# RobotLocomotion/pytorch-dense-correspondence

Hardware: NVIDIA H100
Metric: image-pairs/s (640x480, D=3) fwd+loss+bwd (higher is better)
Workload: dtype f32 (bf16x3 split on the wgmma tensor cores, fp32 accumulate)

## Files before the change

### pytorch-dense-correspondence_b200/csrc/conv_tc.cu

```cuda
#include <cuda.h>
#include <algorithm>
#include <cstring>
#include <functional>
#include <mutex>
#include <unordered_map>

#include "conv.cuh"
#include "conv_tc.cuh"

namespace ddn {

constexpr int TC_BLOCK_K = 64;
constexpr int TC_CONSUMERS = 256;
constexpr int TC_THREADS = TC_CONSUMERS + 32;
constexpr int TC_PRODUCER_WARP = TC_CONSUMERS / 32;
constexpr int TC_WIDE_THREADS = TC_CONSUMERS + 128;
constexpr int TC_A_BYTES = 128 * TC_BLOCK_K * 2;

__device__ __forceinline__ uint32_t smem_u32(const void* p) { return (uint32_t)__cvta_generic_to_shared(p); }

__device__ __forceinline__ void mbar_init(uint32_t bar, uint32_t count) {
  asm volatile("mbarrier.init.shared::cta.b64 [%0], %1;" ::"r"(bar), "r"(count));
}
__device__ __forceinline__ void mbar_expect_tx(uint32_t bar, uint32_t bytes) {
// ... 24 lines not shown
  asm volatile(
      "cp.async.bulk.tensor.2d.shared::cluster.global.mbarrier::complete_tx::bytes [%0], [%1, {%3, %4}], [%2];"
      ::"r"(dst), "l"(map), "r"(bar), "r"(c0), "r"(c1) : "memory");
}
__device__ __forceinline__ void tma_prefetch_l2_4d(const CUtensorMap* map, int c0, int c1, int c2, int c3) {
  asm volatile("cp.async.bulk.prefetch.tensor.4d.L2.global.tile [%0, {%1, %2, %3, %4}];" ::"l"(map), "r"(c0), "r"(c1), "r"(c2), "r"(c3) : "memory");
}
__device__ __forceinline__ void tma_prefetch_desc(const CUtensorMap* map) {
  asm volatile("prefetch.tensormap [%0];" ::"l"(map) : "memory");
}

__device__ __forceinline__ uint64_t gmma_desc(uint32_t smem_addr, uint32_t lbo_bytes, uint32_t sbo_bytes) {
  return (uint64_t)((smem_addr >> 4) & 0x3FFF) | ((uint64_t)((lbo_bytes >> 4) & 0x3FFF) << 16) |
         ((uint64_t)((sbo_bytes >> 4) & 0x3FFF) << 32) | ((uint64_t)1 << 62);
}
__device__ __forceinline__ uint64_t gmma_desc_k(uint32_t smem_addr, uint32_t sbo_bytes = 1024) { return gmma_desc(smem_addr, 16, sbo_bytes); }

template <int R>
__device__ __forceinline__ void setmaxnreg_dec() { asm volatile("setmaxnreg.dec.sync.aligned.u32 %0;" ::"n"(R)); }
template <int R>
__device__ __forceinline__ void setmaxnreg_inc() { asm volatile("setmaxnreg.inc.sync.aligned.u32 %0;" ::"n"(R)); }
__device__ __forceinline__ void wgmma_fence() { asm volatile("wgmma.fence.sync.aligned;" ::: "memory"); }
__device__ __forceinline__ void wgmma_commit() { asm volatile("wgmma.commit_group.sync.aligned;" ::: "memory"); }
template <int N>
__device__ __forceinline__ void wgmma_wait() { asm volatile("wgmma.wait_group.sync.aligned %0;" ::"n"(N) : "memory"); }
template <int K>
__device__ __forceinline__ void fence_acc(float (&d)[K]) {
#pragma unroll
  for (int i = 0; i < K; ++i) asm volatile("" : "+f"(d[i])::"memory");
}

template <int N> struct Wgmma;
template <> struct Wgmma<32> {
  template <int TRANS>
  static __device__ __forceinline__ void mma(float (&d)[16], uint64_t a, uint64_t b, int scale_d) {
    asm volatile(
        "{\n.reg .pred p;\nsetp.ne.b32 p, %18, 0;\n"
        "wgmma.mma_async.sync.aligned.m64n32k16.f32.bf16.bf16 {"
        "%0, %1, %2, %3, %4, %5, %6, %7, %8, %9, %10, %11, %12, %13, %14, %15"
        "}, %16, %17, p, 1, 1, %19, %19;\n}\n"
        : "+f"(d[0]), "+f"(d[1]), "+f"(d[2]), "+f"(d[3]), "+f"(d[4]), "+f"(d[5]), "+f"(d[6]), "+f"(d[7]),
          "+f"(d[8]), "+f"(d[9]), "+f"(d[10]), "+f"(d[11]), "+f"(d[12]), "+f"(d[13]), "+f"(d[14]), "+f"(d[15])
        : "l"(a), "l"(b), "r"(scale_d), "n"(TRANS));
  }
};
template <> struct Wgmma<64> {
  template <int TRANS>
  static __device__ __forceinline__ void mma(float (&d)[32], uint64_t a, uint64_t b, int scale_d) {
    asm volatile(
        "{\n.reg .pred p;\nsetp.ne.b32 p, %34, 0;\n"
        "wgmma.mma_async.sync.aligned.m64n64k16.f32.bf16.bf16 {"
        "%0, %1, %2, %3, %4, %5, %6, %7, %8, %9, %10, %11, %12, %13, %14, %15, "
        "%16, %17, %18, %19, %20, %21, %22, %23, %24, %25, %26, %27, %28, %29, %30, %31"
        "}, %32, %33, p, 1, 1, %35, %35;\n}\n"
        : "+f"(d[0]), "+f"(d[1]), "+f"(d[2]), "+f"(d[3]), "+f"(d[4]), "+f"(d[5]), "+f"(d[6]), "+f"(d[7]),
          "+f"(d[8]), "+f"(d[9]), "+f"(d[10]), "+f"(d[11]), "+f"(d[12]), "+f"(d[13]), "+f"(d[14]), "+f"(d[15]),
          "+f"(d[16]), "+f"(d[17]), "+f"(d[18]), "+f"(d[19]), "+f"(d[20]), "+f"(d[21]), "+f"(d[22]), "+f"(d[23]),
          "+f"(d[24]), "+f"(d[25]), "+f"(d[26]), "+f"(d[27]), "+f"(d[28]), "+f"(d[29]), "+f"(d[30]), "+f"(d[31])
        : "l"(a), "l"(b), "r"(scale_d), "n"(TRANS));
  }
};
template <> struct Wgmma<128> {
  template <int TRANS>
  static __device__ __forceinline__ void mma(float (&d)[64], uint64_t a, uint64_t b, int scale_d) {
    asm volatile(
        "{\n.reg .pred p;\nsetp.ne.b32 p, %66, 0;\n"
        "wgmma.mma_async.sync.aligned.m64n128k16.f32.bf16.bf16 {"
        "%0, %1, %2, %3, %4, %5, %6, %7, %8, %9, %10, %11, %12, %13, %14, %15, "
        "%16, %17, %18, %19, %20, %21, %22, %23, %24, %25, %26, %27, %28, %29, %30, %31, "
        "%32, %33, %34, %35, %36, %37, %38, %39, %40, %41, %42, %43, %44, %45, %46, %47, "
        "%48, %49, %50, %51, %52, %53, %54, %55, %56, %57, %58, %59, %60, %61, %62, %63"
        "}, %64, %65, p, 1, 1, %67, %67;\n}\n"
        : "+f"(d[0]), "+f"(d[1]), "+f"(d[2]), "+f"(d[3]), "+f"(d[4]), "+f"(d[5]), "+f"(d[6]), "+f"(d[7]),
          "+f"(d[8]), "+f"(d[9]), "+f"(d[10]), "+f"(d[11]), "+f"(d[12]), "+f"(d[13]), "+f"(d[14]), "+f"(d[15]),
          "+f"(d[16]), "+f"(d[17]), "+f"(d[18]), "+f"(d[19]), "+f"(d[20]), "+f"(d[21]), "+f"(d[22]), "+f"(d[23]),
          "+f"(d[24]), "+f"(d[25]), "+f"(d[26]), "+f"(d[27]), "+f"(d[28]), "+f"(d[29]), "+f"(d[30]), "+f"(d[31]),
          "+f"(d[32]), "+f"(d[33]), "+f"(d[34]), "+f"(d[35]), "+f"(d[36]), "+f"(d[37]), "+f"(d[38]), "+f"(d[39]),
          "+f"(d[40]), "+f"(d[41]), "+f"(d[42]), "+f"(d[43]), "+f"(d[44]), "+f"(d[45]), "+f"(d[46]), "+f"(d[47]),
          "+f"(d[48]), "+f"(d[49]), "+f"(d[50]), "+f"(d[51]), "+f"(d[52]), "+f"(d[53]), "+f"(d[54]), "+f"(d[55]),
          "+f"(d[56]), "+f"(d[57]), "+f"(d[58]), "+f"(d[59]), "+f"(d[60]), "+f"(d[61]), "+f"(d[62]), "+f"(d[63])
        : "l"(a), "l"(b), "r"(scale_d), "n"(TRANS));
  }
};

template <int N, int TRANS, int NPROD>
__device__ __forceinline__ void mma_k16(float (&d)[N / 2], uint64_t a_hi, uint64_t a_lo, uint64_t b_hi, uint64_t b_lo, int accumulate) {
  if (NPROD == 3) {
    Wgmma<N>::template mma<TRANS>(d, a_hi, b_lo, accumulate);
    Wgmma<N>::template mma<TRANS>(d, a_lo, b_hi, 1);
    Wgmma<N>::template mma<TRANS>(d, a_hi, b_hi, 1);
  } else {
    Wgmma<N>::template mma<TRANS>(d, a_hi, b_hi, accumulate);
  }
}
template <int N, int TRANS, int NPROD>
__device__ __forceinline__ void mma_k16_x(float (&d)[N / 2], float (&x)[N / 2], uint64_t a_hi, uint64_t a_lo, uint64_t b_hi, uint64_t b_lo,
                                          int accumulate) {
  if (NPROD == 3) {
    Wgmma<N>::template mma<TRANS>(x, a_hi, b_lo, accumulate);
    Wgmma<N>::template mma<TRANS>(x, a_lo, b_hi, 1);
  }
  Wgmma<N>::template mma<TRANS>(d, a_hi, b_hi, accumulate);
}
template <int K>
__device__ __forceinline__ void add_cross(float (&d)[K], const float (&x)[K]) {
#pragma unroll
  for (int i = 0; i < K; ++i) d[i] += x[i];
}
template <int N, int K>
__device__ __forceinline__ float (&acc_cols(float (&d)[K]))[N / 2] {
  static_assert(N / 2 <= K, "accumulator too narrow");
  return *reinterpret_cast<float(*)[N / 2]>(&d[0]);
}

constexpr int EPI_ROWS = 4;
constexpr int EPI_STRIDE = 40;
constexpr int EPI_WARP_FLOATS = 16 * EPI_STRIDE;

template <int K>
__device__ __forceinline__ void stage_write(const float (&acc)[K], int c, float* st, int lane) {
  const int r = lane >> 2, q = (lane & 3) * 2;
#pragma unroll
  for (int jj = 0; jj < 4; ++jj) {
    const int j = 4 * c + jj;
    *reinterpret_cast<float2*>(st + r * EPI_STRIDE + 8 * jj + q) = make_float2(acc[4 * j], acc[4 * j + 1]);
    *reinterpret_cast<float2*>(st + (r + 8) * EPI_STRIDE + 8 * jj + q) = make_float2(acc[4 * j + 2], acc[4 * j + 3]);
  }
  __syncwarp();
}

template <int K>
__device__ __forceinline__ void stage_chunk(const float (&acc)[K], int c, float* st, int lane, float4 (&v)[EPI_ROWS]) {
  stage_write(acc, c, st, lane);
  const int ga = lane >> 3, gb = lane & 7;
#pragma unroll
  for (int i = 0; i < EPI_ROWS; ++i) v[i] = *reinterpret_cast<const float4*>(st + (EPI_ROWS * ga + i) * EPI_STRIDE + 4 * gb);
  __syncwarp();
}

__device__ __forceinline__ uint32_t pack_bf16x2(__nv_bfloat16 a, __nv_bfloat16 b) {
  return (uint32_t)__bfloat16_as_ushort(a) | ((uint32_t)__bfloat16_as_ushort(b) << 16);
}

struct TcEpilogueParams {
  float* out;
  const float* addend;
  int imgs_per_group;
  BnFwdFinal fin;
  TcBwdStats bst;
  const float* ep_scale; const float* ep_shift; int ep_relu;
  __nv_bfloat16* out_hi; __nv_bfloat16* out_lo;
};

__device__ __forceinline__ void conv_epilogue_rows(const TcEpilogueParams& p, const float4 (&v)[EPI_ROWS], size_t off, size_t rs, int n_ok, int ch,
                                                   int C, int grp, float4& s1, float4& s2) {
  float4 adv[EPI_ROWS];
#pragma unroll
  for (int i = 0; i < EPI_ROWS; ++i)
    adv[i] = (p.addend && i < n_ok) ? __ldg(reinterpret_cast<const float4*>(p.addend + off + i * rs)) : make_float4(0.f, 0.f, 0.f, 0.f);
  if (p.ep_scale) {
    const float4 sc = __ldg(reinterpret_cast<const float4*>(p.ep_scale + ch));
    const float4 sh = __ldg(reinterpret_cast<const float4*>(p.ep_shift + ch));
#pragma unroll
    for (int i = 0; i < EPI_ROWS; ++i) {
      float4 f = make_float4(fmaf(v[i].x, sc.x, sh.x) + adv[i].x, fmaf(v[i].y, sc.y, sh.y) + adv[i].y,
                             fmaf(v[i].z, sc.z, sh.z) + adv[i].z, fmaf(v[i].w, sc.w, sh.w) + adv[i].w);
      if (p.ep_relu) { f.x = fmaxf(f.x, 0.f); f.y = fmaxf(f.y, 0.f); f.z = fmaxf(f.z, 0.f); f.w = fmaxf(f.w, 0.f); }
      if (i < n_ok) {
        if (p.out) *reinterpret_cast<float4*>(p.out + off + i * rs) = f;
        if (p.out_hi) {
          const __nv_bfloat16 h0 = __float2bfloat16_rn(f.x), h1 = __float2bfloat16_rn(f.y), h2 = __float2bfloat16_rn(f.z), h3 = __float2bfloat16_rn(f.w);
          *reinterpret_cast<uint2*>(p.out_hi + off + i * rs) = make_uint2(pack_bf16x2(h0, h1), pack_bf16x2(h2, h3));
          if (p.out_lo)
            *reinterpret_cast<uint2*>(p.out_lo + off + i * rs) =
                make_uint2(pack_bf16x2(__float2bfloat16_rn(f.x - __bfloat162float(h0)), __float2bfloat16_rn(f.y - __bfloat162float(h1))),
                           pack_bf16x2(__float2bfloat16_rn(f.z - __bfloat162float(h2)), __float2bfloat16_rn(f.w - __bfloat162float(h3))));
        }
      }
    }
  } else if (p.bst.fin.a.acc) {
    float4 rw[EPI_ROWS];
    uint2 yh[EPI_ROWS];
#pragma unroll
    for (int i = 0; i < EPI_ROWS; ++i) {
      rw[i] = i < n_ok ? __ldg(reinterpret_cast<const float4*>(p.bst.raw + off + i * rs)) : make_float4(0.f, 0.f, 0.f, 0.f);
      if (p.bst.y_hi) yh[i] = i < n_ok ? __ldg(reinterpret_cast<const uint2*>(p.bst.y_hi + off + i * rs)) : make_uint2(0u, 0u);
    }
    const float4 mu = __ldg(reinterpret_cast<const float4*>(p.bst.mean + (size_t)grp * C + ch));
    const float4 is = __ldg(reinterpret_cast<const float4*>(p.bst.invstd + (size_t)grp * C + ch));
    float4 scl = make_float4(0.f, 0.f, 0.f, 0.f), be = scl;
    if (!p.bst.y_hi && p.bst.relu) {
      const float4 gm = __ldg(reinterpret_cast<const float4*>(p.bst.gamma + ch));
      be = __ldg(reinterpret_cast<const float4*>(p.bst.beta + ch));
      scl = make_float4(gm.x * is.x, gm.y * is.y, gm.z * is.z, gm.w * is.w);
    }
#pragma unroll
    for (int i = 0; i < EPI_ROWS; ++i) {
      float4 g = make_float4(v[i].x + adv[i].x, v[i].y + adv[i].y, v[i].z + adv[i].z, v[i].w + adv[i].w);
      if (i < n_ok) *reinterpret_cast<float4*>(p.out + off + i * rs) = g;
      else g = make_float4(0.f, 0.f, 0.f, 0.f);
      if (p.bst.y_hi) {
        const uint2 hh = yh[i];
        if ((hh.x & 0x8000u) || !(hh.x & 0x7fffu)) g.x = 0.f;
        if ((hh.x & 0x80000000u) || !(hh.x & 0x7fff0000u)) g.y = 0.f;
        if ((hh.y & 0x8000u) || !(hh.y & 0x7fffu)) g.z = 0.f;
        if ((hh.y & 0x80000000u) || !(hh.y & 0x7fff0000u)) g.w = 0.f;
      } else if (p.bst.relu) {
        if (!(fmaf(rw[i].x - mu.x, scl.x, be.x) > 0.f)) g.x = 0.f;
        if (!(fmaf(rw[i].y - mu.y, scl.y, be.y) > 0.f)) g.y = 0.f;
        if (!(fmaf(rw[i].z - mu.z, scl.z, be.z) > 0.f)) g.z = 0.f;
        if (!(fmaf(rw[i].w - mu.w, scl.w, be.w) > 0.f)) g.w = 0.f;
      }
      s1.x += g.x; s1.y += g.y; s1.z += g.z; s1.w += g.w;
      s2.x = fmaf(g.x, (rw[i].x - mu.x) * is.x, s2.x); s2.y = fmaf(g.y, (rw[i].y - mu.y) * is.y, s2.y);
      s2.z = fmaf(g.z, (rw[i].z - mu.z) * is.z, s2.z); s2.w = fmaf(g.w, (rw[i].w - mu.w) * is.w, s2.w);
    }
  } else {
#pragma unroll
    for (int i = 0; i < EPI_ROWS; ++i) {
      const float4 raw = i < n_ok ? v[i] : make_float4(0.f, 0.f, 0.f, 0.f);
      if (i < n_ok)
        *reinterpret_cast<float4*>(p.out + off + i * rs) = make_float4(raw.x + adv[i].x, raw.y + adv[i].y, raw.z + adv[i].z, raw.w + adv[i].w);
      s1.x += raw.x; s1.y += raw.y; s1.z += raw.z; s1.w += raw.w;
      s2.x = fmaf(raw.x, raw.x, s2.x); s2.y = fmaf(raw.y, raw.y, s2.y); s2.z = fmaf(raw.z, raw.z, s2.z); s2.w = fmaf(raw.w, raw.w, s2.w);
    }
  }
}

__device__ __forceinline__ void colsum_lane_groups(float4& s1, float4& s2) {
#pragma unroll
  for (int off = 8; off < 32; off <<= 1) {
    s1.x += __shfl_xor_sync(0xffffffffu, s1.x, off); s1.y += __shfl_xor_sync(0xffffffffu, s1.y, off);
    s1.z += __shfl_xor_sync(0xffffffffu, s1.z, off); s1.w += __shfl_xor_sync(0xffffffffu, s1.w, off);
    s2.x += __shfl_xor_sync(0xffffffffu, s2.x, off); s2.y += __shfl_xor_sync(0xffffffffu, s2.y, off);
    s2.z += __shfl_xor_sync(0xffffffffu, s2.z, off); s2.w += __shfl_xor_sync(0xffffffffu, s2.w, off);
  }
}

__device__ __forceinline__ void named_barrier(int id, int threads) { asm volatile("bar.sync %0, %1;" ::"r"(id), "r"(threads) : "memory"); }

__device__ __forceinline__ void conv_epilogue_finalize(const TcEpilogueParams& p, int C, int* s_last, int bar) {
  if (p.fin.a.acc) {
    if (bn_last_cta(p.fin.a.ticket, gridDim.x, threadIdx.x == 0, s_last, [bar] { named_barrier(bar, TC_CONSUMERS); }))
      for (int c = threadIdx.x; c < C; c += TC_CONSUMERS) bn_fwd_finalize_channel(p.fin, c);
  } else if (p.bst.fin.a.acc) {
    if (bn_last_cta(p.bst.fin.a.ticket, gridDim.x, threadIdx.x == 0, s_last, [bar] { named_barrier(bar, TC_CONSUMERS); }))
      for (int c = threadIdx.x; c < C; c += TC_CONSUMERS) bn_bwd_finalize_channel(p.bst.fin, c);
  }
}

struct TcConvParams {
  TcEpilogueParams epi;
  int N, H, W, Cin, Cout;
  int taps_w;
  int dil;
  int stride;
  int tiles_h, tiles_w;
  int n_sub;
  int n_co;
  int full_items, tail_split, total_items;
};

constexpr int TC_SUB_H = 4, TC_SUB_W = 16;
constexpr int TC_SUB_BYTES = 64 * 128;

struct TcItem { int sp, co0, width; };
__device__ __forceinline__ TcItem tc_item(const TcConvParams& p, int idx, int block_n) {
  int tile = idx, piece = 0, width = block_n;
  if (idx >= p.full_items) {
    const int j = idx - p.full_items;
    tile = p.full_items + j / p.tail_split;
    piece = j - (j / p.tail_split) * p.tail_split;
    width = block_n / p.tail_split;
  }
  TcItem it;
  it.sp = tile / p.n_co;
  it.co0 = (tile - it.sp * p.n_co) * block_n + piece * width;
  it.width = width;
  return it;
}
struct TcSub { int n, h0, w0; bool valid; };
__device__ __forceinline__ TcSub tc_sub(const TcConvParams& p, int st) {
  TcSub s;
  s.valid = st < p.n_sub;
  const int tw = st % p.tiles_w; const int t = st / p.tiles_w;
  const int th = t % p.tiles_h;
  s.n = s.valid ? t / p.tiles_h : p.N;
  s.h0 = th * TC_SUB_H; s.w0 = tw * TC_SUB_W;
  return s;
}

template <int W, int BLOCK_N, int NPROD, int STAGES, int TRANS = 0>
__device__ __forceinline__ void conv_tc_mainloop(float (&acc)[W / 2], float (&accx)[W / 2], int num_kb, uint32_t& g, const uint64_t* full_bar,
                                                 const uint64_t* empty_bar, const uint8_t* smem, int wg, int lane) {
  constexpr int NSPLIT = NPROD == 3 ? 2 : 1;
  constexpr int A_BYTES = 128 * TC_BLOCK_K * 2;
  constexpr int B_BYTES = BLOCK_N * TC_BLOCK_K * 2;
  constexpr int STAGE_BYTES = NSPLIT * (A_BYTES + B_BYTES);
  constexpr uint32_t LBO = TRANS ? TC_SUB_BYTES : 16;
  constexpr int K_STEP = TRANS ? 16 * 128 : 32;
  for (int kb = 0; kb < num_kb; ++kb, ++g) {
    const int s = g % STAGES;
    mbar_wait(smem_u32(&full_bar[s]), (g / STAGES) & 1);
    wgmma_fence();
    const uint32_t stg = smem_u32(smem + (size_t)s * STAGE_BYTES);
    const uint64_t a_hi = gmma_desc(stg + wg * TC_SUB_BYTES, LBO, 1024), a_lo = gmma_desc(stg + A_BYTES + wg * TC_SUB_BYTES, LBO, 1024);
    const uint64_t b_hi = gmma_desc(stg + NSPLIT * A_BYTES, LBO, 1024), b_lo = gmma_desc(stg + 2 * A_BYTES + B_BYTES, LBO, 1024);
#pragma unroll
    for (int k = 0; k < TC_BLOCK_K / 16; ++k) {
      const uint64_t adv = (uint64_t)((k * K_STEP) >> 4);
      mma_k16_x<W, TRANS, NPROD>(acc, accx, a_hi + adv, a_lo + adv, b_hi + adv, b_lo + adv, (kb | k) != 0);
    }
    wgmma_commit();
    wgmma_wait<1>();
    if (kb > 0 && lane == 0) mbar_arrive(smem_u32(&empty_bar[(g - 1) % STAGES]));
  }
  wgmma_wait<0>();
  fence_acc(acc);
  if (NPROD == 3) { fence_acc(accx); add_cross(acc, accx); }
  if (lane == 0) mbar_arrive(smem_u32(&empty_bar[(g - 1) % STAGES]));
}

template <int BLOCK_N, int NPROD>
__global__ void __launch_bounds__(TC_WIDE_THREADS, 1)
conv_tc_kernel(const __grid_constant__ CUtensorMap tm_a_hi, const __grid_constant__ CUtensorMap tm_a_lo,
               const __grid_constant__ CUtensorMap tm_b_hi, const __grid_constant__ CUtensorMap tm_b_lo,
               const __grid_constant__ CUtensorMap tm_bt_hi, const __grid_constant__ CUtensorMap tm_bt_lo,
               const TcConvParams p) {
  constexpr int NSPLIT = NPROD == 3 ? 2 : 1;
  constexpr int A_BYTES = 128 * TC_BLOCK_K * 2;
  constexpr int B_BYTES = BLOCK_N * TC_BLOCK_K * 2;
  constexpr int STAGE_BYTES = NSPLIT * (A_BYTES + B_BYTES);
  constexpr int STAGES = (192 * 1024) / STAGE_BYTES >= 8 ? 8 : (192 * 1024) / STAGE_BYTES;
  static_assert(STAGES >= 2, "pipeline needs at least two stages");

  extern __shared__ __align__(1024) uint8_t smem_raw[];
  uint8_t* smem = reinterpret_cast<uint8_t*>((reinterpret_cast<uintptr_t>(smem_raw) + 1023) & ~uintptr_t(1023));
  __shared__ __align__(8) uint64_t full_bar[STAGES];
  __shared__ __align__(8) uint64_t empty_bar[STAGES];
  __shared__ int s_last;
  __shared__ __align__(16) float s_stage[TC_CONSUMERS / 32][EPI_WARP_FLOATS];
  __shared__ __align__(16) float s_part[2][2][4][BLOCK_N];

  pdl_trigger();
  const int warp = __shfl_sync(0xffffffffu, threadIdx.x >> 5, 0), lane = threadIdx.x & 31;
  const int cin_chunks = p.Cin / TC_BLOCK_K;
  const int num_kb = p.taps_w * p.taps_w * cin_chunks;
  const int half = p.taps_w >> 1;

  if (threadIdx.x == 0) {
    for (int s = 0; s < STAGES; ++s) { mbar_init(smem_u32(&full_bar[s]), 1); mbar_init(smem_u32(&empty_bar[s]), TC_CONSUMERS / 32); }
    fence_barrier_init();
    tma_prefetch_desc(&tm_a_hi); tma_prefetch_desc(&tm_b_hi); tma_prefetch_desc(&tm_bt_hi);
    if (NSPLIT == 2) { tma_prefetch_desc(&tm_a_lo); tma_prefetch_desc(&tm_b_lo); tma_prefetch_desc(&tm_bt_lo); }
  }
  __syncthreads();
  pdl_wait();

  if (warp >= TC_PRODUCER_WARP) {
    setmaxnreg_dec<40>();
    if (warp == TC_PRODUCER_WARP && lane == 0) {
      uint32_t g = 0;
      for (int idx = blockIdx.x; idx < p.total_items; idx += gridDim.x) {
        const TcItem it = tc_item(p, idx, BLOCK_N);
        const bool tail = it.width != BLOCK_N;
        const uint32_t stage_tx = (uint32_t)(NSPLIT * (A_BYTES + it.width * TC_BLOCK_K * 2));
        const CUtensorMap* mb_hi = tail ? &tm_bt_hi : &tm_b_hi;
        const CUtensorMap* mb_lo = tail ? &tm_bt_lo : &tm_b_lo;
        const TcSub s0 = tc_sub(p, it.sp * 2), s1 = tc_sub(p, it.sp * 2 + 1);
        for (int kb = 0; kb < num_kb; ++kb, ++g) {
          const int s = g % STAGES;
          mbar_wait(smem_u32(&empty_bar[s]), ((g / STAGES) & 1) ^ 1);
          const int tap = kb / cin_chunks, cc = kb - tap * cin_chunks;
          const int r = tap / p.taps_w, sx = tap - r * p.taps_w;
          const int dh = (r - half) * p.dil, dw = (sx - half) * p.dil;
          uint8_t* stg = smem + (size_t)s * STAGE_BYTES;
          const uint32_t bar = smem_u32(&full_bar[s]);
          mbar_expect_tx(bar, stage_tx);
          tma_load_4d(smem_u32(stg), &tm_a_hi, bar, cc * TC_BLOCK_K, s0.w0 * p.stride + dw, s0.h0 * p.stride + dh, s0.n);
          tma_load_4d(smem_u32(stg + TC_SUB_BYTES), &tm_a_hi, bar, cc * TC_BLOCK_K, s1.w0 * p.stride + dw, s1.h0 * p.stride + dh, s1.n);
          tma_load_2d(smem_u32(stg + NSPLIT * A_BYTES), mb_hi, bar, kb * TC_BLOCK_K, it.co0);
          if (NSPLIT == 2) {
            tma_load_4d(smem_u32(stg + A_BYTES), &tm_a_lo, bar, cc * TC_BLOCK_K, s0.w0 * p.stride + dw, s0.h0 * p.stride + dh, s0.n);
            tma_load_4d(smem_u32(stg + A_BYTES + TC_SUB_BYTES), &tm_a_lo, bar, cc * TC_BLOCK_K, s1.w0 * p.stride + dw, s1.h0 * p.stride + dh, s1.n);
            tma_load_2d(smem_u32(stg + 2 * A_BYTES + B_BYTES), mb_lo, bar, kb * TC_BLOCK_K, it.co0);
          }
        }
      }
    }
  } else {
    setmaxnreg_inc<232>();
    const int wg = warp >> 2, w = warp & 3, e = threadIdx.x & 127;
    const int ga = lane >> 3, gb = lane & 7;
    const bool stats = p.epi.fin.a.acc != nullptr;
    const bool bstats = p.epi.bst.fin.a.acc != nullptr;
    double* const sum_acc = bstats ? p.epi.bst.fin.a.acc : p.epi.fin.a.acc;
    float* const st = s_stage[warp];
    float acc[BLOCK_N / 2], accx[BLOCK_N / 2];
    uint32_t g = 0;
    for (int idx = blockIdx.x; idx < p.total_items; idx += gridDim.x) {
      const TcItem it = tc_item(p, idx, BLOCK_N);
      if (it.width == BLOCK_N)
        conv_tc_mainloop<BLOCK_N, BLOCK_N, NPROD, STAGES>(acc, accx, num_kb, g, full_bar, empty_bar, smem, wg, lane);
      else if (BLOCK_N > 64 && it.width == 64)
        conv_tc_mainloop<64, BLOCK_N, NPROD, STAGES>(acc_cols<64>(acc), acc_cols<64>(accx), num_kb, g, full_bar, empty_bar, smem, wg, lane);
      else
        conv_tc_mainloop<32, BLOCK_N, NPROD, STAGES>(acc_cols<32>(acc), acc_cols<32>(accx), num_kb, g, full_bar, empty_bar, smem, wg, lane);

      const TcSub sb = tc_sub(p, it.sp * 2 + wg);
      const int h = sb.h0 + w, w4 = sb.w0 + EPI_ROWS * ga;
      const int n_ok = (sb.valid && h < p.H) ? min(EPI_ROWS, p.W - w4) : 0;
      const size_t pix = ((size_t)(n_ok > 0 ? sb.n : 0) * p.H + (n_ok > 0 ? h : 0)) * p.W + (n_ok > 0 ? w4 : 0);
      const size_t cbase = pix * p.Cout + it.co0 + gb * 4;
      const int grp = sb.valid ? sb.n / p.epi.imgs_per_group : 0;
#pragma unroll
      for (int c = 0; c < BLOCK_N / 32; ++c) {
        if (c < (it.width >> 5)) {
          float4 v[EPI_ROWS];
          stage_chunk(acc, c, st, lane, v);
          float4 s1 = make_float4(0.f, 0.f, 0.f, 0.f), s2 = s1;
          conv_epilogue_rows(p.epi, v, cbase + c * 32, (size_t)p.Cout, n_ok, it.co0 + c * 32 + gb * 4, p.Cout, grp, s1, s2);
          if (stats || bstats) {
            colsum_lane_groups(s1, s2);
            if (ga == 0) {
              *reinterpret_cast<float4*>(&s_part[wg][0][w][c * 32 + gb * 4]) = s1;
              *reinterpret_cast<float4*>(&s_part[wg][1][w][c * 32 + gb * 4]) = s2;
            }
          }
        }
      }
      if (stats || bstats) {
        named_barrier(1 + wg, 128);
        if (sb.valid)
          for (int col = e; col < it.width; col += 128) {
#pragma unroll
            for (int k = 0; k < 2; ++k) {
              const float sum = s_part[wg][k][0][col] + s_part[wg][k][1][col] + s_part[wg][k][2][col] + s_part[wg][k][3][col];
              red_add_f64(sum_acc + (size_t)(grp * 2 + k) * p.Cout + it.co0 + col, (double)sum);
            }
          }
        named_barrier(1 + wg, 128);
      }
    }
    conv_epilogue_finalize(p.epi, p.Cout, &s_last, 3);
  }
}

struct TcHaloParams {
  TcEpilogueParams epi;
  int N, H, W;
  int tiles_h, tiles_w, n_tiles;
};
constexpr int HALO_TH = 8, HALO_TW = 16;
constexpr int HALO_BH = HALO_TH + 2, HALO_BW = HALO_TW + 2;
constexpr int HALO_BOX_BYTES = HALO_BH * HALO_BW * 128;
constexpr int HALO_SLOT = ((HALO_BOX_BYTES + 1023) / 1024) * 1024;
constexpr int HALO_B_TAP = 64 * 128;
constexpr int HALO_B_PLANE = 9 * HALO_B_TAP;
__host__ __device__ constexpr int halo_slots(int nprod) { return nprod == 3 ? 2 : 3; }

template <int NPROD>
__global__ void __launch_bounds__(TC_THREADS, 1)
conv64_halo_kernel(const __grid_constant__ CUtensorMap tm_a_hi, const __grid_constant__ CUtensorMap tm_a_lo,
                   const __grid_constant__ CUtensorMap tm_b_hi, const __grid_constant__ CUtensorMap tm_b_lo, const TcHaloParams p) {
  constexpr int NSPLIT = NPROD == 3 ? 2 : 1;
  constexpr int SLOTS = halo_slots(NPROD);
  extern __shared__ __align__(1024) uint8_t smem_raw[];
  uint8_t* smem = reinterpret_cast<uint8_t*>((reinterpret_cast<uintptr_t>(smem_raw) + 1023) & ~uintptr_t(1023));
  uint8_t* smem_b = smem;
  uint8_t* smem_a = smem + NSPLIT * HALO_B_PLANE;
  __shared__ __align__(8) uint64_t full_bar[SLOTS], empty_bar[SLOTS], b_full;
  __shared__ int s_last;
  __shared__ __align__(16) float s_stage[TC_CONSUMERS / 32][EPI_WARP_FLOATS];
  __shared__ __align__(16) float s_part[2][8][64];

  pdl_trigger();
  const int warp = __shfl_sync(0xffffffffu, threadIdx.x >> 5, 0), lane = threadIdx.x & 31;
  if (threadIdx.x == 0) {
    for (int s = 0; s < SLOTS; ++s) { mbar_init(smem_u32(&full_bar[s]), 1); mbar_init(smem_u32(&empty_bar[s]), TC_CONSUMERS / 32); }
    mbar_init(smem_u32(&b_full), 1);
    fence_barrier_init();
    tma_prefetch_desc(&tm_a_hi); tma_prefetch_desc(&tm_b_hi);
    if (NSPLIT == 2) { tma_prefetch_desc(&tm_a_lo); tma_prefetch_desc(&tm_b_lo); }
  }
  __syncthreads();
  pdl_wait();

  auto tile_of = [&](int t, int& n, int& h0, int& w0) {
    const int tw = t % p.tiles_w; const int q = t / p.tiles_w;
    const int th = q % p.tiles_h; n = q / p.tiles_h;
    h0 = th * HALO_TH; w0 = tw * HALO_TW;
  };

  if (warp == TC_PRODUCER_WARP) {
    if (lane == 0) {
      const uint32_t bb = smem_u32(&b_full);
      mbar_expect_tx(bb, NSPLIT * HALO_B_PLANE);
#pragma unroll 1
      for (int tap = 0; tap < 9; ++tap) {
        tma_load_2d(smem_u32(smem_b + tap * HALO_B_TAP), &tm_b_hi, bb, tap * 64, 0);
        if (NSPLIT == 2) tma_load_2d(smem_u32(smem_b + HALO_B_PLANE + tap * HALO_B_TAP), &tm_b_lo, bb, tap * 64, 0);
      }
      uint32_t g = 0;
      constexpr int PF = 2;
      for (int j = 0; j < PF; ++j) {
        const int tp = blockIdx.x + j * gridDim.x;
        if (tp < p.n_tiles) {
          int n, h0, w0;
          tile_of(tp, n, h0, w0);
          tma_prefetch_l2_4d(&tm_a_hi, 0, h0 - 1, w0 - 1, n);
          if (NSPLIT == 2) tma_prefetch_l2_4d(&tm_a_lo, 0, h0 - 1, w0 - 1, n);
        }
      }
      for (int t = blockIdx.x; t < p.n_tiles; t += gridDim.x) {
        int n, h0, w0;
        {
          const int tp = t + PF * gridDim.x;
          if (tp < p.n_tiles) {
            tile_of(tp, n, h0, w0);
            tma_prefetch_l2_4d(&tm_a_hi, 0, h0 - 1, w0 - 1, n);
            if (NSPLIT == 2) tma_prefetch_l2_4d(&tm_a_lo, 0, h0 - 1, w0 - 1, n);
          }
        }
        tile_of(t, n, h0, w0);
#pragma unroll
        for (int pl = 0; pl < NSPLIT; ++pl, ++g) {
          const int s = g % SLOTS;
          mbar_wait(smem_u32(&empty_bar[s]), ((g / SLOTS) & 1) ^ 1);
          const uint32_t bar = smem_u32(&full_bar[s]);
          mbar_expect_tx(bar, HALO_BOX_BYTES);
          tma_load_4d(smem_u32(smem_a + s * HALO_SLOT), pl == 0 ? &tm_a_hi : &tm_a_lo, bar, 0, h0 - 1, w0 - 1, n);
        }
      }
    }
  } else {
    const int wg = warp >> 2, w = warp & 3;
    const int ga = lane >> 3, gb = lane & 7;
    const bool stats = p.epi.fin.a.acc != nullptr;
    const bool bstats = p.epi.bst.fin.a.acc != nullptr;
    double* const sum_acc = bstats ? p.epi.bst.fin.a.acc : p.epi.fin.a.acc;
    float* const st = s_stage[warp];
    mbar_wait(smem_u32(&b_full), 0);
    const uint64_t bd_hi = gmma_desc_k(smem_u32(smem_b));
    const uint64_t bd_lo = gmma_desc_k(smem_u32(smem_b + HALO_B_PLANE));
    const uint32_t a_wg = (uint32_t)(8 * wg * HALO_BH * 128);
    float acc[32], accx[32];
    uint32_t g = 0;
    for (int t = blockIdx.x; t < p.n_tiles; t += gridDim.x) {
      int n, h0, w0;
      tile_of(t, n, h0, w0);
      const int s_hi = g % SLOTS;
      {
        mbar_wait(smem_u32(&full_bar[s_hi]), (g / SLOTS) & 1);
        wgmma_fence();
        const uint64_t a0 = gmma_desc_k(smem_u32(smem_a + s_hi * HALO_SLOT) + a_wg, HALO_BH * 128);
#pragma unroll
        for (int tap = 0; tap < 9; ++tap) {
#pragma unroll
          for (int k = 0; k < 4; ++k) {
            const uint64_t ad = a0 + (uint64_t)((((tap % 3) * HALO_BH + tap / 3) * 128 + k * 32) >> 4);
            const uint64_t boff = (uint64_t)((tap * HALO_B_TAP + k * 32) >> 4);
            if (NPROD == 3) Wgmma<64>::mma<0>(accx, ad, bd_lo + boff, (tap | k) != 0);
            Wgmma<64>::mma<0>(acc, ad, bd_hi + boff, (tap | k) != 0);
          }
        }
        wgmma_commit();
        ++g;
      }
      if (NPROD == 3) {
        const int s = g % SLOTS;
        mbar_wait(smem_u32(&full_bar[s]), (g / SLOTS) & 1);
        const uint64_t a0 = gmma_desc_k(smem_u32(smem_a + s * HALO_SLOT) + a_wg, HALO_BH * 128);
#pragma unroll
        for (int tap = 0; tap < 9; ++tap) {
#pragma unroll
          for (int k = 0; k < 4; ++k)
            Wgmma<64>::mma<0>(accx, a0 + (uint64_t)((((tap % 3) * HALO_BH + tap / 3) * 128 + k * 32) >> 4),
                              bd_hi + (uint64_t)((tap * HALO_B_TAP + k * 32) >> 4), 1);
        }
        wgmma_commit();
        wgmma_wait<1>();
        if (lane == 0) mbar_arrive(smem_u32(&empty_bar[s_hi]));
        ++g;
      }
      wgmma_wait<0>();
      fence_acc(acc);
      if (NPROD == 3) { fence_acc(accx); add_cross(acc, accx); }
      if (lane == 0) mbar_arrive(smem_u32(&empty_bar[(g - 1) % SLOTS]));

      const size_t pix0 = ((size_t)n * p.H + h0 + EPI_ROWS * (ga & 1)) * p.W + (w0 + 8 * wg + 2 * w + (ga >> 1));
      const size_t row_stride = (size_t)p.W * 64;
      const int grp = n / p.epi.imgs_per_group;
#pragma unroll
      for (int c = 0; c < 2; ++c) {
        float4 v[EPI_ROWS];
        stage_chunk(acc, c, st, lane, v);
        float4 s1 = make_float4(0.f, 0.f, 0.f, 0.f), s2 = s1;
        conv_epilogue_rows(p.epi, v, pix0 * 64 + gb * 4 + c * 32, row_stride, EPI_ROWS, c * 32 + gb * 4, 64, grp, s1, s2);
        if (stats || bstats) {
          colsum_lane_groups(s1, s2);
          if (ga == 0) {
            *reinterpret_cast<float4*>(&s_part[0][warp][c * 32 + gb * 4]) = s1;
            *reinterpret_cast<float4*>(&s_part[1][warp][c * 32 + gb * 4]) = s2;
          }
        }
      }
      if (stats || bstats) {
        named_barrier(3, TC_CONSUMERS);
        if (threadIdx.x < 128) {
          const int col = threadIdx.x & 63, k = threadIdx.x >> 6;
          float s8 = 0.f;
#pragma unroll
          for (int q = 0; q < 8; ++q) s8 += s_part[k][q][col];
          red_add_f64(sum_acc + (size_t)(grp * 2 + k) * 64 + col, (double)s8);
        }
        named_barrier(3, TC_CONSUMERS);
      }
    }
    conv_epilogue_finalize(p.epi, 64, &s_last, 3);
  }
}

struct TcWgradParams {
  double* dwp;
  int N, H, W, Cin, Cout;
  int taps_w, dil, stride;
  int tiles_h, tiles_w;
  int total_kb;
  int n_co, n_ci, n_tiles;
  int chunks;
};

struct WgradItem { int co0, ci0, tap, kb0, kb1; };
__device__ __forceinline__ WgradItem wgrad_item(const TcWgradParams& p, int idx, int bn) {
  const int c = idx / p.n_tiles;
  int t = idx - c * p.n_tiles;
  WgradItem it;
  it.co0 = (t % p.n_co) * 128; t /= p.n_co;
  it.ci0 = (t % p.n_ci) * bn;
  it.tap = t / p.n_ci;
  it.kb0 = (int)((int64_t)c * p.total_kb / p.chunks);
  it.kb1 = (int)((int64_t)(c + 1) * p.total_kb / p.chunks);
  return it;
}

template <int BN, int NPROD>
__global__ void __launch_bounds__(TC_WIDE_THREADS, 1)
wgrad_tc_kernel(const __grid_constant__ CUtensorMap tm_dy_hi, const __grid_constant__ CUtensorMap tm_dy_lo,
                const __grid_constant__ CUtensorMap tm_x_hi, const __grid_constant__ CUtensorMap tm_x_lo,
                const TcWgradParams p) {
  constexpr int NSPLIT = NPROD == 3 ? 2 : 1;
  constexpr int B_BYTES = BN * TC_BLOCK_K * 2;
  constexpr int STAGE_BYTES = NSPLIT * (TC_A_BYTES + B_BYTES);
  constexpr int STAGES = (192 * 1024) / STAGE_BYTES >= 8 ? 8 : (192 * 1024) / STAGE_BYTES;
  static_assert(STAGES >= 2, "pipeline needs at least two stages");

  extern __shared__ __align__(1024) uint8_t smem_raw[];
  uint8_t* smem = reinterpret_cast<uint8_t*>((reinterpret_cast<uintptr_t>(smem_raw) + 1023) & ~uintptr_t(1023));
  __shared__ __align__(8) uint64_t full_bar[STAGES];
  __shared__ __align__(8) uint64_t empty_bar[STAGES];
  __shared__ __align__(16) float s_stage[TC_CONSUMERS / 32][EPI_WARP_FLOATS];

  pdl_trigger();
  const int warp = __shfl_sync(0xffffffffu, threadIdx.x >> 5, 0), lane = threadIdx.x & 31;
  const int total_items = p.chunks * p.n_tiles;
  const int half = p.taps_w >> 1;

  if (threadIdx.x == 0) {
    for (int s = 0; s < STAGES; ++s) { mbar_init(smem_u32(&full_bar[s]), 1); mbar_init(smem_u32(&empty_bar[s]), TC_CONSUMERS / 32); }
    fence_barrier_init();
    tma_prefetch_desc(&tm_dy_hi); tma_prefetch_desc(&tm_x_hi);
    if (NSPLIT == 2) { tma_prefetch_desc(&tm_dy_lo); tma_prefetch_desc(&tm_x_lo); }
  }
  __syncthreads();
  pdl_wait();

  if (warp >= TC_PRODUCER_WARP) {
    setmaxnreg_dec<40>();
    if (warp == TC_PRODUCER_WARP && lane == 0) {
      uint32_t g = 0;
      for (int idx = blockIdx.x; idx < total_items; idx += gridDim.x) {
        const WgradItem it = wgrad_item(p, idx, BN);
        const int r = it.tap / p.taps_w, sx = it.tap - r * p.taps_w;
        const int dh = (r - half) * p.dil, dw = (sx - half) * p.dil;
        for (int kb = it.kb0; kb < it.kb1; ++kb, ++g) {
          const int s = g % STAGES;
          mbar_wait(smem_u32(&empty_bar[s]), ((g / STAGES) & 1) ^ 1);
          const int tw = kb % p.tiles_w, q = kb / p.tiles_w;
          const int th = q % p.tiles_h, n = q / p.tiles_h;
          const int h0 = th * TC_SUB_H, w0 = tw * TC_SUB_W;
          const int hh = h0 * p.stride + dh, ww = w0 * p.stride + dw;
          uint8_t* stg = smem + (size_t)s * STAGE_BYTES;
          const uint32_t bar = smem_u32(&full_bar[s]);
          mbar_expect_tx(bar, STAGE_BYTES);
#pragma unroll
          for (int hf = 0; hf < 2; ++hf) {
            tma_load_4d(smem_u32(stg + hf * TC_SUB_BYTES), &tm_dy_hi, bar, it.co0 + 64 * hf, w0, h0, n);
            if (NSPLIT == 2) tma_load_4d(smem_u32(stg + TC_A_BYTES + hf * TC_SUB_BYTES), &tm_dy_lo, bar, it.co0 + 64 * hf, w0, h0, n);
          }
#pragma unroll
          for (int part = 0; part < BN / 64; ++part) {
            tma_load_4d(smem_u32(stg + NSPLIT * TC_A_BYTES + part * TC_SUB_BYTES), &tm_x_hi, bar, it.ci0 + 64 * part, ww, hh, n);
            if (NSPLIT == 2)
              tma_load_4d(smem_u32(stg + 2 * TC_A_BYTES + B_BYTES + part * TC_SUB_BYTES), &tm_x_lo, bar, it.ci0 + 64 * part, ww, hh, n);
          }
        }
      }
    }
  } else {
    setmaxnreg_inc<232>();
    const int wg = warp >> 2, w = warp & 3;
    float* const st = s_stage[warp];
    float acc[BN / 2], accx[BN / 2];
    uint32_t g = 0;
    for (int idx = blockIdx.x; idx < total_items; idx += gridDim.x) {
      const WgradItem it = wgrad_item(p, idx, BN);
      if (it.co0 + 64 * wg >= p.Cout) {
        for (int kb = it.kb0; kb < it.kb1; ++kb, ++g) {
          mbar_wait(smem_u32(&full_bar[g % STAGES]), (g / STAGES) & 1);
          if (lane == 0) mbar_arrive(smem_u32(&empty_bar[g % STAGES]));
        }
      } else {
        conv_tc_mainloop<BN, BN, NPROD, STAGES, 1>(acc, accx, it.kb1 - it.kb0, g, full_bar, empty_bar, smem, wg, lane);
        double* const dst = p.dwp + ((size_t)it.tap * p.Cout + it.co0 + 64 * wg + 16 * w) * p.Cin + it.ci0 + lane;
#pragma unroll
        for (int c = 0; c < BN / 32; ++c) {
          stage_write(acc, c, st, lane);
#pragma unroll
          for (int i = 0; i < 16; ++i) red_add_f64(dst + (size_t)i * p.Cin + 32 * c, (double)st[i * EPI_STRIDE + lane]);
          __syncwarp();
        }
      }
    }
  }
}

struct TcWgradHaloParams {
  double* dwp;
  int N, H, W;
  int tiles_h, tiles_w, n_tiles;
};
constexpr int WGH_CONSUMERS = 384;
constexpr int WGH_THREADS = WGH_CONSUMERS + 32;
constexpr int WGH_X_SLOT = HALO_SLOT;
constexpr int WGH_DY_BYTES = 128 * 128;
__host__ __device__ constexpr int wgh_off(int tap) { return (tap % 3) * HALO_BH + tap / 3; }

template <int NPROD>
__global__ void __launch_bounds__(WGH_THREADS, 1)
wgrad64_halo_kernel(const __grid_constant__ CUtensorMap tm_x_hi, const __grid_constant__ CUtensorMap tm_x_lo,
                    const __grid_constant__ CUtensorMap tm_dy_hi, const __grid_constant__ CUtensorMap tm_dy_lo, const TcWgradHaloParams p) {
  constexpr int NSPLIT = NPROD == 3 ? 2 : 1;
  constexpr int STAGE = NSPLIT * (WGH_X_SLOT + WGH_DY_BYTES);
  constexpr int STAGES = 2;
  extern __shared__ __align__(1024) uint8_t smem_raw[];
  uint8_t* smem = reinterpret_cast<uint8_t*>((reinterpret_cast<uintptr_t>(smem_raw) + 1023) & ~uintptr_t(1023));
  __shared__ __align__(8) uint64_t full_bar[STAGES], empty_bar[STAGES];

  pdl_trigger();
  const int warp = __shfl_sync(0xffffffffu, threadIdx.x >> 5, 0), lane = threadIdx.x & 31;
  if (threadIdx.x == 0) {
    for (int s = 0; s < STAGES; ++s) { mbar_init(smem_u32(&full_bar[s]), 1); mbar_init(smem_u32(&empty_bar[s]), WGH_CONSUMERS / 32); }
    fence_barrier_init();
    tma_prefetch_desc(&tm_x_hi); tma_prefetch_desc(&tm_dy_hi);
    if (NSPLIT == 2) { tma_prefetch_desc(&tm_x_lo); tma_prefetch_desc(&tm_dy_lo); }
  }
  __syncthreads();
  pdl_wait();
  const int my_tiles = p.n_tiles > (int)blockIdx.x ? (p.n_tiles - (int)blockIdx.x + (int)gridDim.x - 1) / (int)gridDim.x : 0;
  if (my_tiles == 0) return;

  if (warp == WGH_CONSUMERS / 32) {
    if (lane == 0) {
      int i = 0;
      for (int t = blockIdx.x; t < p.n_tiles; t += gridDim.x, ++i) {
        const int tw = t % p.tiles_w; const int q = t / p.tiles_w;
        const int th = q % p.tiles_h, n = q / p.tiles_h;
        const int h0 = th * HALO_TH, w0 = tw * HALO_TW;
        const int s = i % STAGES;
        mbar_wait(smem_u32(&empty_bar[s]), ((i / STAGES) & 1) ^ 1);
        const uint32_t bar = smem_u32(&full_bar[s]);
        mbar_expect_tx(bar, NSPLIT * (HALO_BOX_BYTES + WGH_DY_BYTES));
        uint8_t* stg = smem + (size_t)s * STAGE;
        tma_load_4d(smem_u32(stg), &tm_x_hi, bar, 0, h0 - 1, w0 - 1, n);
        tma_load_4d(smem_u32(stg + NSPLIT * WGH_X_SLOT), &tm_dy_hi, bar, 0, h0, w0, n);
        if (NSPLIT == 2) {
          tma_load_4d(smem_u32(stg + WGH_X_SLOT), &tm_x_lo, bar, 0, h0 - 1, w0 - 1, n);
          tma_load_4d(smem_u32(stg + NSPLIT * WGH_X_SLOT + WGH_DY_BYTES), &tm_dy_lo, bar, 0, h0, w0, n);
        }
      }
    }
  } else {
    const int r = warp >> 2, w = warp & 3;
    float acc[3][32];
    for (int i = 0; i < my_tiles; ++i) {
      const int s = i % STAGES;
      mbar_wait(smem_u32(&full_bar[s]), (i / STAGES) & 1);
      wgmma_fence();
      const uint32_t stg = smem_u32(smem + (size_t)s * STAGE);
      const uint32_t x_hi = stg, x_lo = stg + WGH_X_SLOT;
      const uint32_t d_hi = stg + NSPLIT * WGH_X_SLOT, d_lo = d_hi + WGH_DY_BYTES;
      const uint64_t b_hi0 = gmma_desc(d_hi, 1024, 1024);
      const uint64_t b_lo0 = gmma_desc(d_lo, 1024, 1024);
#pragma unroll
      for (int sx = 0; sx < 3; ++sx) {
        const int oa = wgh_off(r * 3 + sx);
        const uint64_t a_hi0 = gmma_desc(x_hi + oa * 128, 1024, HALO_BH * 128);
        const uint64_t a_lo0 = gmma_desc(x_lo + oa * 128, 1024, HALO_BH * 128);
#pragma unroll
        for (int kk = 0; kk < 8; ++kk) {
          const uint64_t a_adv = (uint64_t)((2 * kk * HALO_BH * 128) >> 4);
          const uint64_t b_adv = (uint64_t)((kk * 16 * 128) >> 4);
          mma_k16<64, 1, NPROD>(acc[sx], a_hi0 + a_adv, a_lo0 + a_adv, b_hi0 + b_adv, b_lo0 + b_adv, (i | kk) != 0);
        }
      }
      wgmma_commit();
      wgmma_wait<1>();
      if (i > 0 && lane == 0) mbar_arrive(smem_u32(&empty_bar[(i - 1) % STAGES]));
    }
    wgmma_wait<0>();
#pragma unroll
    for (int sx = 0; sx < 3; ++sx) fence_acc(acc[sx]);
    const int ci = 16 * w + (lane >> 2), co = 2 * (lane & 3);
#pragma unroll
    for (int sx = 0; sx < 3; ++sx) {
      double* dst = p.dwp + (size_t)(r * 3 + sx) * 64 * 64;
#pragma unroll
      for (int j = 0; j < 8; ++j) {
        red_add_f64(dst + (size_t)(co + 8 * j) * 64 + ci, (double)acc[sx][4 * j]);
        red_add_f64(dst + (size_t)(co + 8 * j + 1) * 64 + ci, (double)acc[sx][4 * j + 1]);
        red_add_f64(dst + (size_t)(co + 8 * j) * 64 + ci + 8, (double)acc[sx][4 * j + 2]);
        red_add_f64(dst + (size_t)(co + 8 * j + 1) * 64 + ci + 8, (double)acc[sx][4 * j + 3]);
      }
    }
  }
}

__global__ void unpack_wgrad_tc_kernel(const double* __restrict__ dwp, float* __restrict__ dw, int Cout, int Cin, int taps) {
  pdl_prologue();
  const int64_t total = (int64_t)Cout * Cin * taps;
  for (int64_t i = (int64_t)blockIdx.x * blockDim.x + threadIdx.x; i < total; i += (int64_t)gridDim.x * blockDim.x) {
    int tap = (int)(i % taps); int64_t q = i / taps;
    int ci = (int)(q % Cin); int co = (int)(q / Cin);
    dw[i] = (float)dwp[((int64_t)tap * Cout + co) * Cin + ci];
  }
}

__global__ void unpack_wgrad_batched_kernel(const double* __restrict__ dwp_base, float* __restrict__ grads_base, TcUnpackTable t) {
  pdl_prologue();
  const TcUnpackEntry en = t.e[blockIdx.y];
  const double* __restrict__ dwp = dwp_base + en.src_off;
  float* __restrict__ dw = grads_base + en.dst_off;
  if (en.kind == 1) {
    for (int i = blockIdx.x * blockDim.x + threadIdx.x; i < 64 * 147; i += gridDim.x * blockDim.x) {
      const int rs = i % 49, c = (i / 49) % 3, co = i / 147;
      dw[i] = (float)dwp[co * 192 + rs * 3 + c];
    }
    return;
  }
  const int64_t total = (int64_t)en.Cout * en.Cin * en.taps;
  for (int64_t i = (int64_t)blockIdx.x * blockDim.x + threadIdx.x; i < total; i += (int64_t)gridDim.x * blockDim.x) {
    int tap = (int)(i % en.taps); int64_t q = i / en.taps;
    int ci = (int)(q % en.Cin); int co = (int)(q / en.Cin);
    dw[i] = (float)dwp[((int64_t)tap * en.Cout + co) * en.Cin + ci];
  }
}

__global__ void split_bf16_kernel(const float* __restrict__ x, __nv_bfloat16* __restrict__ hi, __nv_bfloat16* __restrict__ lo,
                                  int64_t n4, int want_lo) {
  pdl_prologue();
  for (int64_t i = (int64_t)blockIdx.x * blockDim.x + threadIdx.x; i < n4; i += (int64_t)gridDim.x * blockDim.x) {
    float4 v = __ldg(reinterpret_cast<const float4*>(x) + i);
    __nv_bfloat16 h0 = __float2bfloat16_rn(v.x), h1 = __float2bfloat16_rn(v.y), h2 = __float2bfloat16_rn(v.z), h3 = __float2bfloat16_rn(v.w);
    __nv_bfloat162 a = __halves2bfloat162(h0, h1), b = __halves2bfloat162(h2, h3);
    uint2 ho; ho.x = *reinterpret_cast<uint32_t*>(&a); ho.y = *reinterpret_cast<uint32_t*>(&b);
    reinterpret_cast<uint2*>(hi)[i] = ho;
// ... 659 lines not shown
```

Before: 141.5.

## Overlap epilogue operand loads with final wgmma and prefetch halo epilogue data

Splits the conv epilogue into a load phase and a compute phase. The addend, raw and y_hi operand loads for the first chunk are issued while the last wgmma group is still in flight, and the next chunk's loads are double-buffered across the epilogue loop. The halo kernel also issues L2 prefetches for its epilogue operands at tile start. The aim is to hide global-load latency in the epilogue, at the cost of extra registers held live during the mainloop and an added zeroing of accx.

```diff
diff --git a/pytorch-dense-correspondence_b200/csrc/conv_tc.cu b/pytorch-dense-correspondence_b200/csrc/conv_tc.cu
--- a/pytorch-dense-correspondence_b200/csrc/conv_tc.cu
+++ b/pytorch-dense-correspondence_b200/csrc/conv_tc.cu
@@ -200,12 +200,43 @@
   __nv_bfloat16* out_hi; __nv_bfloat16* out_lo;
 };
 
-__device__ __forceinline__ void conv_epilogue_rows(const TcEpilogueParams& p, const float4 (&v)[EPI_ROWS], size_t off, size_t rs, int n_ok, int ch,
-                                                   int C, int grp, float4& s1, float4& s2) {
+struct TcEpilogueOperands {
   float4 adv[EPI_ROWS];
+  float4 rw[EPI_ROWS];
+  uint2 yh[EPI_ROWS];
+};
+
+__device__ __forceinline__ void conv_epilogue_load(const TcEpilogueParams& p, size_t off, size_t rs, int n_ok, TcEpilogueOperands& o) {
 #pragma unroll
   for (int i = 0; i < EPI_ROWS; ++i)
-    adv[i] = (p.addend && i < n_ok) ? __ldg(reinterpret_cast<const float4*>(p.addend + off + i * rs)) : make_float4(0.f, 0.f, 0.f, 0.f);
+    o.adv[i] = (p.addend && i < n_ok) ? __ldg(reinterpret_cast<const float4*>(p.addend + off + i * rs)) : make_float4(0.f, 0.f, 0.f, 0.f);
+  const bool bst = !p.ep_scale && p.bst.fin.a.acc;
+#pragma unroll
+  for (int i = 0; i < EPI_ROWS; ++i) {
+    o.rw[i] = (bst && i < n_ok) ? __ldg(reinterpret_cast<const float4*>(p.bst.raw + off + i * rs)) : make_float4(0.f, 0.f, 0.f, 0.f);
+    o.yh[i] = (bst && p.bst.y_hi && i < n_ok) ? __ldg(reinterpret_cast<const uint2*>(p.bst.y_hi + off + i * rs)) : make_uint2(0u, 0u);
+  }
+}
+
+__device__ __forceinline__ void prefetch_l2(const void* ptr) { asm volatile("prefetch.global.L2 [%0];" ::"l"(ptr)); }
+
+__device__ __forceinline__ void conv_epilogue_prefetch(const TcEpilogueParams& p, size_t off0, size_t rs, int n_ok, int chunks, int gb) {
+  if (gb >= chunks) return;
+  const size_t off = off0 + (size_t)gb * 32;
+  const bool bst = !p.ep_scale && p.bst.fin.a.acc;
+#pragma unroll
+  for (int i = 0; i < EPI_ROWS; ++i) {
+    if (i < n_ok) {
+      if (p.addend) prefetch_l2(p.addend + off + i * rs);
+      if (bst) prefetch_l2(p.bst.raw + off + i * rs);
+      if (bst && p.bst.y_hi && !(gb & 1)) prefetch_l2(p.bst.y_hi + off + i * rs);
+    }
+  }
+}
+
+__device__ __forceinline__ void conv_epilogue_rows(const TcEpilogueParams& p, const TcEpilogueOperands& o, const float4 (&v)[EPI_ROWS],
+                                                   size_t off, size_t rs, int n_ok, int ch, int C, int grp, float4& s1, float4& s2) {
+  const float4 (&adv)[EPI_ROWS] = o.adv;
   if (p.ep_scale) {
     const float4 sc = __ldg(reinterpret_cast<const float4*>(p.ep_scale + ch));
     const float4 sh = __ldg(reinterpret_cast<const float4*>(p.ep_shift + ch));
@@ -227,13 +258,8 @@
       }
     }
   } else if (p.bst.fin.a.acc) {
-    float4 rw[EPI_ROWS];
-    uint2 yh[EPI_ROWS];
-#pragma unroll
-    for (int i = 0; i < EPI_ROWS; ++i) {
-      rw[i] = i < n_ok ? __ldg(reinterpret_cast<const float4*>(p.bst.raw + off + i * rs)) : make_float4(0.f, 0.f, 0.f, 0.f);
-      if (p.bst.y_hi) yh[i] = i < n_ok ? __ldg(reinterpret_cast<const uint2*>(p.bst.y_hi + off + i * rs)) : make_uint2(0u, 0u);
-    }
+    const float4 (&rw)[EPI_ROWS] = o.rw;
+    const uint2 (&yh)[EPI_ROWS] = o.yh;
     const float4 mu = __ldg(reinterpret_cast<const float4*>(p.bst.mean + (size_t)grp * C + ch));
     const float4 is = __ldg(reinterpret_cast<const float4*>(p.bst.invstd + (size_t)grp * C + ch));
     float4 scl = make_float4(0.f, 0.f, 0.f, 0.f), be = scl;
@@ -338,9 +364,9 @@
   return s;
 }
 
-template <int W, int BLOCK_N, int NPROD, int STAGES, int TRANS = 0>
+template <int W, int BLOCK_N, int NPROD, int STAGES, int TRANS = 0, class UnderLast>
 __device__ __forceinline__ void conv_tc_mainloop(float (&acc)[W / 2], float (&accx)[W / 2], int num_kb, uint32_t& g, const uint64_t* full_bar,
-                                                 const uint64_t* empty_bar, const uint8_t* smem, int wg, int lane) {
+                                                 const uint64_t* empty_bar, const uint8_t* smem, int wg, int lane, UnderLast&& under_last) {
   constexpr int NSPLIT = NPROD == 3 ? 2 : 1;
   constexpr int A_BYTES = 128 * TC_BLOCK_K * 2;
   constexpr int B_BYTES = BLOCK_N * TC_BLOCK_K * 2;
@@ -363,6 +389,7 @@
     wgmma_wait<1>();
     if (kb > 0 && lane == 0) mbar_arrive(smem_u32(&empty_bar[(g - 1) % STAGES]));
   }
+  under_last();
   wgmma_wait<0>();
   fence_acc(acc);
   if (NPROD == 3) { fence_acc(accx); add_cross(acc, accx); }
@@ -448,26 +475,36 @@
     uint32_t g = 0;
     for (int idx = blockIdx.x; idx < p.total_items; idx += gridDim.x) {
       const TcItem it = tc_item(p, idx, BLOCK_N);
-      if (it.width == BLOCK_N)
-        conv_tc_mainloop<BLOCK_N, BLOCK_N, NPROD, STAGES>(acc, accx, num_kb, g, full_bar, empty_bar, smem, wg, lane);
-      else if (BLOCK_N > 64 && it.width == 64)
-        conv_tc_mainloop<64, BLOCK_N, NPROD, STAGES>(acc_cols<64>(acc), acc_cols<64>(accx), num_kb, g, full_bar, empty_bar, smem, wg, lane);
-      else
-        conv_tc_mainloop<32, BLOCK_N, NPROD, STAGES>(acc_cols<32>(acc), acc_cols<32>(accx), num_kb, g, full_bar, empty_bar, smem, wg, lane);
-
       const TcSub sb = tc_sub(p, it.sp * 2 + wg);
       const int h = sb.h0 + w, w4 = sb.w0 + EPI_ROWS * ga;
       const int n_ok = (sb.valid && h < p.H) ? min(EPI_ROWS, p.W - w4) : 0;
       const size_t pix = ((size_t)(n_ok > 0 ? sb.n : 0) * p.H + (n_ok > 0 ? h : 0)) * p.W + (n_ok > 0 ? w4 : 0);
       const size_t cbase = pix * p.Cout + it.co0 + gb * 4;
       const int grp = sb.valid ? sb.n / p.epi.imgs_per_group : 0;
+      TcEpilogueOperands ops[2];
+      auto load_chunk = [&](int c) {
+        conv_epilogue_load(p.epi, cbase + c * 32, (size_t)p.Cout, n_ok, ops[c & 1]);
+      };
+      auto load_first = [&] { load_chunk(0); };
+#pragma unroll
+      for (int i = 0; i < BLOCK_N / 2; ++i) accx[i] = 0.f;
+      if (it.width == BLOCK_N)
+        conv_tc_mainloop<BLOCK_N, BLOCK_N, NPROD, STAGES>(acc, accx, num_kb, g, full_bar, empty_bar, smem, wg, lane, load_first);
+      else if (BLOCK_N > 64 && it.width == 64)
+        conv_tc_mainloop<64, BLOCK_N, NPROD, STAGES>(acc_cols<64>(acc), acc_cols<64>(accx), num_kb, g, full_bar, empty_bar, smem, wg, lane,
+                                                     load_first);
+      else
+        conv_tc_mainloop<32, BLOCK_N, NPROD, STAGES>(acc_cols<32>(acc), acc_cols<32>(accx), num_kb, g, full_bar, empty_bar, smem, wg, lane,
+                                                     load_first);
+
 #pragma unroll
       for (int c = 0; c < BLOCK_N / 32; ++c) {
         if (c < (it.width >> 5)) {
           float4 v[EPI_ROWS];
           stage_chunk(acc, c, st, lane, v);
+          if (c + 1 < (it.width >> 5)) load_chunk(c + 1);
           float4 s1 = make_float4(0.f, 0.f, 0.f, 0.f), s2 = s1;
-          conv_epilogue_rows(p.epi, v, cbase + c * 32, (size_t)p.Cout, n_ok, it.co0 + c * 32 + gb * 4, p.Cout, grp, s1, s2);
+          conv_epilogue_rows(p.epi, ops[c & 1], v, cbase + c * 32, (size_t)p.Cout, n_ok, it.co0 + c * 32 + gb * 4, p.Cout, grp, s1, s2);
           if (stats || bstats) {
             colsum_lane_groups(s1, s2);
             if (ga == 0) {
@@ -597,6 +634,14 @@
     for (int t = blockIdx.x; t < p.n_tiles; t += gridDim.x) {
       int n, h0, w0;
       tile_of(t, n, h0, w0);
+      const size_t pix0 = ((size_t)n * p.H + h0 + EPI_ROWS * (ga & 1)) * p.W + (w0 + 8 * wg + 2 * w + (ga >> 1));
+      const size_t row_stride = (size_t)p.W * 64;
+      const int grp = n / p.epi.imgs_per_group;
+      TcEpilogueOperands ops[2];
+      auto load_chunk = [&](int c) {
+        conv_epilogue_load(p.epi, pix0 * 64 + gb * 4 + c * 32, row_stride, EPI_ROWS, ops[c]);
+      };
+      conv_epilogue_prefetch(p.epi, pix0 * 64, row_stride, EPI_ROWS, 2, gb);
       const int s_hi = g % SLOTS;
       {
         mbar_wait(smem_u32(&full_bar[s_hi]), (g / SLOTS) & 1);
@@ -614,6 +659,7 @@
         }
         wgmma_commit();
         ++g;
+        if (NPROD != 3) load_chunk(0);
       }
       if (NPROD == 3) {
         const int s = g % SLOTS;
@@ -627,6 +673,7 @@
                               bd_hi + (uint64_t)((tap * HALO_B_TAP + k * 32) >> 4), 1);
         }
         wgmma_commit();
+        load_chunk(0);
         wgmma_wait<1>();
         if (lane == 0) mbar_arrive(smem_u32(&empty_bar[s_hi]));
         ++g;
@@ -636,15 +683,13 @@
       if (NPROD == 3) { fence_acc(accx); add_cross(acc, accx); }
       if (lane == 0) mbar_arrive(smem_u32(&empty_bar[(g - 1) % SLOTS]));
 
-      const size_t pix0 = ((size_t)n * p.H + h0 + EPI_ROWS * (ga & 1)) * p.W + (w0 + 8 * wg + 2 * w + (ga >> 1));
-      const size_t row_stride = (size_t)p.W * 64;
-      const int grp = n / p.epi.imgs_per_group;
 #pragma unroll
       for (int c = 0; c < 2; ++c) {
         float4 v[EPI_ROWS];
         stage_chunk(acc, c, st, lane, v);
+        if (c == 0) load_chunk(1);
         float4 s1 = make_float4(0.f, 0.f, 0.f, 0.f), s2 = s1;
-        conv_epilogue_rows(p.epi, v, pix0 * 64 + gb * 4 + c * 32, row_stride, EPI_ROWS, c * 32 + gb * 4, 64, grp, s1, s2);
+        conv_epilogue_rows(p.epi, ops[c], v, pix0 * 64 + gb * 4 + c * 32, row_stride, EPI_ROWS, c * 32 + gb * 4, 64, grp, s1, s2);
         if (stats || bstats) {
           colsum_lane_groups(s1, s2);
           if (ga == 0) {
@@ -769,7 +814,7 @@
           if (lane == 0) mbar_arrive(smem_u32(&empty_bar[g % STAGES]));
         }
       } else {
-        conv_tc_mainloop<BN, BN, NPROD, STAGES, 1>(acc, accx, it.kb1 - it.kb0, g, full_bar, empty_bar, smem, wg, lane);
+        conv_tc_mainloop<BN, BN, NPROD, STAGES, 1>(acc, accx, it.kb1 - it.kb0, g, full_bar, empty_bar, smem, wg, lane, [] {});
         double* const dst = p.dwp + ((size_t)it.tap * p.Cout + it.co0 + 64 * wg + 16 * w) * p.Cin + it.ci0 + lane;
 #pragma unroll
         for (int c = 0; c < BN / 32; ++c) {
```

Measured after the change: 142.4, median of 6. No clear change (+0.6%).
